# howardlau1999/pytorch-ddp-template

Hardware: NVIDIA H100
Metric: samples/sec (whole box, device-timed, max over ranks) for ResNet-50 DDP at 1/2/4/8 H100 (higher is better)
Workload: dtype bf16; 1 GPU; model=resnet50, global_batch=32, per_gpu_batch=32, image_size=224, parallelism=dp1, loss=mse(dense one-hot target), optimizer=sgd lr1e-3 + clip_grad_norm 1000 + linear warmup/decay, transport=single, cuda_graph=True

## Files before the change

b200ddp/csrc/conv_wgmma.cu:

```cuda
#include "conv.h"

#include <cuda.h>
#include <mutex>
#include <unordered_map>
#include <vector>

#include "drv.h"
#include "tc_primitives.cuh"

namespace b200 {
namespace {
using namespace tc;

constexpr int BLOCK_K = 64;
constexpr int UMMA_K = 16;
constexpr int kThreads = 256;
constexpr int kMmaWarps = 4;
constexpr int kMaxRing = 12;
constexpr int kSlabBytes = 128 * 128;
constexpr int kStagingBytes = 2 * kSlabBytes;
constexpr int kBarrierBytes = 1024;
constexpr int kTrStride = 36;
constexpr int kStatsScratchBytes = 4 * 32 * kTrStride * 4;
__host__ __device__ constexpr int acc_stride(int block_n) { return block_n + 8; }
__host__ __device__ constexpr int acc_bytes(int block_n) { return 128 * acc_stride(block_n) * 4; }

struct TapGemmParams {
  int M_total, Kc, Nc;
  int R, S, pad;
  int mirror;
  int mode;
  int H, W;
  int BH, BI, tiles_h, Wp;
  int num_m_tiles, num_n_tiles;
  int dense_rows;
  int a_chunk_bytes;
  int KC, TB;
  int s_stage_bytes, s_stages, b_slot_bytes, b_stages;
  uint32_t a_tx_bytes;
  int set_base_offset;
  int b_tap_stride;
  int row_mul;
  int b_resident;
  int chunk_stride;
  float* col_stats;
  const __nv_bfloat16* addend;
  const __nv_bfloat16* bn_x;
  const uint8_t* bn_mask;
  const float* bn_mean;
  const float* bn_rstd;
  long long* dbg;
};

__device__ __forceinline__ void tma_load_4d(const CUtensorMap* map, uint64_t* bar, void* smem, int c0, int c1, int c2, int c3) {
  asm volatile(
      "cp.async.bulk.tensor.4d.shared::cluster.global.mbarrier::complete_tx::bytes [%0], [%1, {%3, %4, %5, %6}], [%2];"
      ::"r"(smem_u32(smem)), "l"(reinterpret_cast<uint64_t>(map)), "r"(smem_u32(bar)), "r"(c0), "r"(c1), "r"(c2), "r"(c3) : "memory");
}
__device__ __forceinline__ void bulk_wait_read_all() { asm volatile("cp.async.bulk.wait_group.read 0;" ::: "memory"); }
__device__ __forceinline__ void epi_bar_sync() { asm volatile("bar.sync 1, 128;" ::: "memory"); }

__device__ __forceinline__ uint64_t make_desc_rowoff(uint32_t addr, uint32_t lbo, uint32_t sbo, int set_base_offset) {
  uint64_t d = make_smem_desc(addr, lbo, sbo);
  if (set_base_offset) d |= (uint64_t)((addr >> 7) & 7u) << 49;
  return d;
}

__device__ __forceinline__ bool acc_row_to_dense(const TapGemmParams& p, int i, int* dense) {
  if (p.mode == 2) {
    const int h = i / p.Wp, w = i - h * p.Wp;
    *dense = h * p.W + w;
    return h < p.BH && w < p.W;
  }
  *dense = i;
  return i < p.dense_rows;
}

__device__ __forceinline__ float warp_column_sum32(const float* v, float* tr, int lane) {
#pragma unroll
  for (int q = 0; q < 8; ++q)
    *reinterpret_cast<float4*>(tr + lane * kTrStride + 4 * q) = make_float4(v[4 * q], v[4 * q + 1], v[4 * q + 2], v[4 * q + 3]);
  __syncwarp();
  float s = 0.f;
#pragma unroll
  for (int r = 0; r < 32; ++r) s += tr[r * kTrStride + lane];
  __syncwarp();
  return s;
}

__device__ __forceinline__ bool elect_one() {
  uint32_t pred;
  asm volatile("{\n\t.reg .pred P;\n\telect.sync _|P, 0xFFFFFFFF;\n\tselp.u32 %0, 1, 0, P;\n\t}" : "=r"(pred));
  return pred != 0;
}

template <int BLOCK_N, bool B_MN, int EPI>
__global__ void __launch_bounds__(kThreads, 1)
conv_tap_gemm_kernel(const __grid_constant__ CUtensorMap map_a, const __grid_constant__ CUtensorMap map_b,
                     const __grid_constant__ CUtensorMap map_d, const TapGemmParams p) {
  constexpr int kBBytes = BLOCK_N * BLOCK_K * 2;
  constexpr int kAccStride = acc_stride(BLOCK_N);
  extern __shared__ uint8_t smem_raw[];
  uint8_t* smem = reinterpret_cast<uint8_t*>((reinterpret_cast<uintptr_t>(smem_raw) + 1023) & ~uintptr_t(1023));
  uint8_t* s_ring = smem;
  uint8_t* b_ring = s_ring + p.s_stages * p.s_stage_bytes;
  uint8_t* staging = b_ring + p.b_stages * p.b_slot_bytes;
  [[maybe_unused]] float* stats_scratch = reinterpret_cast<float*>(staging + kStagingBytes);
  float* acc_smem = reinterpret_cast<float*>(staging + kStagingBytes + (EPI != 0 ? kStatsScratchBytes : 0));
  uint64_t* s_full = reinterpret_cast<uint64_t*>(reinterpret_cast<uint8_t*>(acc_smem) + acc_bytes(BLOCK_N));
  uint64_t* s_empty = s_full + kMaxRing;
  uint64_t* b_full = s_empty + kMaxRing;
  uint64_t* b_empty = b_full + kMaxRing;

  const int warp = threadIdx.x >> 5, lane = threadIdx.x & 31;
  const long long t_begin = clock64();
  const int num_tiles = p.num_m_tiles * p.num_n_tiles;
  const int cblocks = p.Kc / BLOCK_K;
  const int taps = p.R * p.S;
  const int chunks_per_tile = cblocks * taps;

  if (warp == 0 && lane == 0) { tma_prefetch_desc(&map_a); tma_prefetch_desc(&map_b); tma_prefetch_desc(&map_d); }
  if (warp == 1) {
    if (lane < kMaxRing) {
      mbar_init(&s_full[lane], (p.mode == 2 || p.b_resident) ? 1 : 2); mbar_init(&s_empty[lane], kMmaWarps);
      mbar_init(&b_full[lane], 1); mbar_init(&b_empty[lane], kMmaWarps);
    }
    asm volatile("fence.mbarrier_init.release.cluster;" ::: "memory");
  }
  __syncthreads();
#define B200_T0 if (dbg) t = clock64();
#define B200_T1(acc) if (dbg) acc += clock64() - t;

  if (warp == 0 || warp == 3) {
    const bool is_a = (warp == 0);
    int ss = 0, bs = 0;
    uint32_t sph = 0, bph = 0;
    long long d_w = 0, d_i = 0, t = 0;
    const bool dbg = p.dbg != nullptr && blockIdx.x == 0;
    if constexpr (!B_MN) {
      if (!is_a && p.b_resident) {
        if (elect_one()) {
          mbar_expect_tx(&b_full[0], (uint32_t)chunks_per_tile * kBBytes);
          int cb_i = 0, r_i = 0, s_i = 0;
          for (int q = 0; q < chunks_per_tile; ++q) {
            tma_load_2d(&map_b, &b_full[0], b_ring + q * kBBytes, (r_i * p.S + s_i) * p.b_tap_stride + cb_i * BLOCK_K, 0);
            if (++s_i == p.S) { s_i = 0; if (++r_i == p.R) { r_i = 0; ++cb_i; } }
          }
        }
        __syncwarp();
      }
    }
    for (int tile = blockIdx.x; tile < num_tiles; tile += gridDim.x) {
      const int mt = tile / p.num_n_tiles, nt = tile - mt * p.num_n_tiles;
      const int n0 = nt * BLOCK_N;
      int img0 = 0, h0 = 0;
      if (p.mode != 0) { img0 = (mt / p.tiles_h) * p.BI; h0 = (mt % p.tiles_h) * p.BH; }
      if (p.mode != 2) {
        if (!is_a && p.b_resident) continue;
        int cb = 0, r = 0, sx = 0;
        for (int q0 = 0; q0 < chunks_per_tile; q0 += p.KC) {
          B200_T0 mbar_wait(&s_empty[ss], sph ^ 1); B200_T1(d_w)
          B200_T0
          if (elect_one()) {
            uint8_t* dst = s_ring + ss * p.s_stage_bytes;
            int cb_i = cb, r_i = r, s_i = sx;
            if (is_a) {
              mbar_expect_tx(&s_full[ss], (uint32_t)p.KC * p.a_tx_bytes);
              for (int j = 0; j < p.KC; ++j) {
                if (p.mode == 0) {
                  tma_load_4d(&map_a, &s_full[ss], dst, cb_i * BLOCK_K, mt * 128, 0, 0);
                } else {
                  const int dh = p.mirror ? p.pad - r_i : r_i - p.pad, dw = p.mirror ? p.pad - s_i : s_i - p.pad;
                  tma_load_4d(&map_a, &s_full[ss], dst, cb_i * BLOCK_K, dw, h0 * p.row_mul + dh, img0);
                }
                dst += p.chunk_stride;
                if (++s_i == p.S) { s_i = 0; if (++r_i == p.R) { r_i = 0; ++cb_i; } }
              }
            } else {
              mbar_expect_tx(&s_full[ss], (uint32_t)p.KC * kBBytes);
              for (int j = 0; j < p.KC; ++j) {
                uint8_t* sb = dst + p.a_chunk_bytes;
                const int bcol = (r_i * p.S + s_i) * p.b_tap_stride;
                if constexpr (!B_MN) {
                  tma_load_2d(&map_b, &s_full[ss], sb, bcol + cb_i * BLOCK_K, n0);
                } else {
#pragma unroll
                  for (int c = 0; c < BLOCK_N / 64; ++c)
                    tma_load_2d(&map_b, &s_full[ss], sb + c * (64 * BLOCK_K * 2), bcol + n0 + 64 * c, cb_i * BLOCK_K);
                }
                dst += p.chunk_stride;
                if (++s_i == p.S) { s_i = 0; if (++r_i == p.R) { r_i = 0; ++cb_i; } }
              }
            }
          }
          __syncwarp();
          for (int j = 0; j < p.KC; ++j) { if (++sx == p.S) { sx = 0; if (++r == p.R) { r = 0; ++cb; } } }
          if (++ss == p.s_stages) { ss = 0; sph ^= 1; }
          B200_T1(d_i)
        }
      } else if (is_a) {
        for (int cb = 0; cb < cblocks; ++cb) {
          B200_T0 mbar_wait(&s_empty[ss], sph ^ 1); B200_T1(d_w)
          B200_T0
          if (elect_one()) {
            mbar_expect_tx(&s_full[ss], p.a_tx_bytes);
            tma_load_4d(&map_a, &s_full[ss], s_ring + ss * p.s_stage_bytes, cb * BLOCK_K, -p.pad, h0 - p.pad, img0);
          }
          __syncwarp();
          if (++ss == p.s_stages) { ss = 0; sph ^= 1; }
          B200_T1(d_i)
        }
      } else {
        for (int cb = 0; cb < cblocks; ++cb) {
          for (int tap0 = 0; tap0 < taps; tap0 += p.TB) {
            B200_T0 mbar_wait(&b_empty[bs], bph ^ 1); B200_T1(d_w)
            B200_T0
            if (elect_one()) {
              mbar_expect_tx(&b_full[bs], (uint32_t)p.TB * kBBytes);
              for (int j = 0; j < p.TB; ++j) {
                uint8_t* sb = b_ring + bs * p.b_slot_bytes + j * kBBytes;
                const int bcol = (tap0 + j) * p.b_tap_stride;
                if constexpr (!B_MN) {
                  tma_load_2d(&map_b, &b_full[bs], sb, bcol + cb * BLOCK_K, n0);
                } else {
#pragma unroll
                  for (int c = 0; c < BLOCK_N / 64; ++c)
                    tma_load_2d(&map_b, &b_full[bs], sb + c * (64 * BLOCK_K * 2), bcol + n0 + 64 * c, cb * BLOCK_K);
                }
              }
            }
            __syncwarp();
            if (++bs == p.b_stages) { bs = 0; bph ^= 1; }
            B200_T1(d_i)
          }
        }
      }
    }
    if (dbg && lane == 0) { p.dbg[is_a ? 0 : 2] = d_w; p.dbg[is_a ? 1 : 3] = d_i; }
  } else if (warp >= 4) {
    constexpr int kTB = B_MN ? 1 : 0;
    constexpr uint32_t kLboB = B_MN ? BLOCK_K * 128 : 16;
    constexpr uint32_t kStepB = B_MN ? UMMA_K * 128 : UMMA_K * 2;
    constexpr uint64_t kHalfA = (64 * 128) >> 4;
    const uint64_t a_desc0 = make_smem_desc(smem_u32(s_ring), 16, 1024);
    const uint64_t b_desc_s0 = make_smem_desc(smem_u32(s_ring), kLboB, 1024);
    const uint64_t b_desc_b0 = make_smem_desc(smem_u32(b_ring), kLboB, 1024);
    const int ew = warp - 4;
    const bool t0 = (ew == 0 && lane == 0);
    int ss = 0, bs = 0;
    uint32_t sph = 0, bph = 0, slab = 0;
    long long d_wf = 0, d_mma = 0, d_ep = 0, t = 0;
    const bool dbg = p.dbg != nullptr && blockIdx.x == 0 && t0;
    [[maybe_unused]] float st_s[BLOCK_N / 32], st_q[BLOCK_N / 32];
    constexpr bool STATS = (EPI != 0);
    [[maybe_unused]] float* tr = stats_scratch + ew * (32 * kTrStride);
    if constexpr (STATS) {
#pragma unroll
      for (int i = 0; i < BLOCK_N / 32; ++i) { st_s[i] = 0.f; st_q[i] = 0.f; }
    }
    if (p.b_resident) mbar_wait(&b_full[0], 0);
    for (int tile = blockIdx.x; tile < num_tiles; tile += gridDim.x) {
      WgAcc<BLOCK_N> acc;
      uint32_t acc_on = 0;
      if (p.mode != 2) {
        for (int q0 = 0; q0 < chunks_per_tile; q0 += p.KC) {
          B200_T0 mbar_wait(&s_full[ss], sph); B200_T1(d_wf)
          B200_T0
          wgmma_fence();
          uint32_t off = (uint32_t)(ss * p.s_stage_bytes);
          for (int j = 0; j < p.KC; ++j) {
            const uint64_t da = a_desc0 + (uint64_t)(off >> 4);
            const uint64_t db = p.b_resident ? b_desc_b0 + (uint64_t)(((uint32_t)(q0 + j) * (uint32_t)kBBytes) >> 4)
                                             : b_desc_s0 + (uint64_t)((off + p.a_chunk_bytes) >> 4);
#pragma unroll
            for (int k = 0; k < BLOCK_K / UMMA_K; ++k) {
              const uint64_t dak = da + (uint64_t)(k * ((UMMA_K * 2) >> 4));
              wgmma_tile<BLOCK_N, 0, kTB>(acc, dak, dak + kHalfA, db + (uint64_t)(k * (kStepB >> 4)), acc_on);
              acc_on = 1;
            }
            off += (uint32_t)p.chunk_stride;
          }
          wgmma_commit();
          wgmma_wait<0>();
          __syncwarp();
          if (lane == 0) mbar_arrive(&s_empty[ss]);
          if (++ss == p.s_stages) { ss = 0; sph ^= 1; }
          B200_T1(d_mma)
        }
      } else {
        for (int cb = 0; cb < cblocks; ++cb) {
          B200_T0 mbar_wait(&s_full[ss], sph); B200_T1(d_wf)
          const uint32_t a_off = (uint32_t)(ss * p.s_stage_bytes);
          for (int tap0 = 0; tap0 < taps; tap0 += p.TB) {
            B200_T0 mbar_wait(&b_full[bs], bph); B200_T1(d_wf)
            B200_T0
            wgmma_fence();
            int r = tap0 / p.S, sx = tap0 - r * p.S;
            for (int j = 0; j < p.TB; ++j) {
              const int rr = p.mirror ? (p.R - 1 - r) : r, sc = p.mirror ? (p.S - 1 - sx) : sx;
              const uint64_t da = make_desc_rowoff(smem_u32(s_ring) + a_off + (uint32_t)(rr * p.Wp + sc) * 128u, 16, 1024, p.set_base_offset);
              const uint64_t db = b_desc_b0 + (uint64_t)((uint32_t)(bs * p.b_slot_bytes + j * kBBytes) >> 4);
#pragma unroll
              for (int k = 0; k < BLOCK_K / UMMA_K; ++k) {
                const uint64_t dak = da + (uint64_t)(k * ((UMMA_K * 2) >> 4));
                wgmma_tile<BLOCK_N, 0, kTB>(acc, dak, dak + kHalfA, db + (uint64_t)(k * (kStepB >> 4)), acc_on);
                acc_on = 1;
              }
              if (++sx == p.S) { sx = 0; ++r; }
            }
            wgmma_commit();
            wgmma_wait<0>();
            __syncwarp();
            if (lane == 0) {
              mbar_arrive(&b_empty[bs]);
              if (tap0 + p.TB >= taps) mbar_arrive(&s_empty[ss]);
            }
            if (++bs == p.b_stages) { bs = 0; bph ^= 1; }
            B200_T1(d_mma)
          }
          if (++ss == p.s_stages) { ss = 0; sph ^= 1; }
        }
      }
      B200_T0
      const int mt = tile / p.num_n_tiles, nt = tile - mt * p.num_n_tiles;
      const int n0 = nt * BLOCK_N;
      int row0;
      if (p.mode == 0) row0 = mt * 128;
      else row0 = (((mt / p.tiles_h) * p.BI) * p.H + (mt % p.tiles_h) * p.BH) * p.W;
      int dense;
      bool valid = acc_row_to_dense(p, ew * 32 + lane, &dense);
      valid = valid && (row0 + dense < p.M_total);
      wg_bar_sync();
      acc_to_smem<BLOCK_N>(acc, acc_smem, kAccStride, threadIdx.x - 128);
      wg_bar_sync();
#pragma unroll
      for (int c = 0; c < BLOCK_N; c += 64) {
        if (n0 + c >= p.Nc) break;
        uint8_t* buf = staging + (slab & 1u) * kSlabBytes;
        const uint32_t buf_s = smem_u32(buf);
#pragma unroll
        for (int half = 0; half < 2; ++half) {
          uint32_t rr[32];
          acc_row_ld32(acc_smem, kAccStride, ew * 32 + lane, c + 32 * half, rr);
          if constexpr (EPI == 1) {
            float sv[32], qv[32];
#pragma unroll
            for (int i = 0; i < 32; ++i) {
              const float v = __bfloat162float(__float2bfloat16_rn(__uint_as_float(rr[i])));
              sv[i] = valid ? v : 0.f;
              qv[i] = sv[i] * sv[i];
            }
            const float cs = warp_column_sum32(sv, tr, lane);
            const float cq = warp_column_sum32(qv, tr, lane);
            const int ci = (c >> 5) + half;
#pragma unroll
            for (int i = 0; i < BLOCK_N / 32; ++i)
              if (i == ci) { st_s[i] += cs; st_q[i] += cq; }
          }
          if constexpr (EPI == 2) {
            const int col0 = n0 + c + 32 * half;
            const size_t grow = (size_t)(row0 + dense);
            float v[32];
#pragma unroll
            for (int i = 0; i < 32; ++i) v[i] = __uint_as_float(rr[i]);
            if (p.addend != nullptr && valid) {
              const uint4* ap = reinterpret_cast<const uint4*>(p.addend + grow * p.Nc + col0);
#pragma unroll
              for (int q = 0; q < 4; ++q) {
                const uint4 raw = __ldg(ap + q);
                const __nv_bfloat162* h = reinterpret_cast<const __nv_bfloat162*>(&raw);
#pragma unroll
                for (int j = 0; j < 4; ++j) { const float2 f = __bfloat1622float2(h[j]); v[8 * q + 2 * j] += f.x; v[8 * q + 2 * j + 1] += f.y; }
              }
            }
#pragma unroll
            for (int i = 0; i < 32; ++i) { v[i] = __bfloat162float(__float2bfloat16_rn(v[i])); rr[i] = __float_as_uint(v[i]); }
            if (p.bn_x != nullptr) {
              float sv[32], qv[32];
              uint32_t mk = 0xffffffffu;
              float xv[32];
              if (valid) {
                const uint4* xp = reinterpret_cast<const uint4*>(p.bn_x + grow * p.Nc + col0);
#pragma unroll
                for (int q = 0; q < 4; ++q) {
                  const uint4 raw = __ldg(xp + q);
                  const __nv_bfloat162* h = reinterpret_cast<const __nv_bfloat162*>(&raw);
#pragma unroll
                  for (int j = 0; j < 4; ++j) { const float2 f = __bfloat1622float2(h[j]); xv[8 * q + 2 * j] = f.x; xv[8 * q + 2 * j + 1] = f.y; }
                }
                if (p.bn_mask != nullptr) mk = __ldg(reinterpret_cast<const uint32_t*>(p.bn_mask + grow * (size_t)(p.Nc >> 3) + (col0 >> 3)));
              } else {
                mk = 0u;
#pragma unroll
                for (int i = 0; i < 32; ++i) xv[i] = 0.f;
              }
              const float my_mean = (col0 + lane < p.Nc) ? __ldg(p.bn_mean + col0 + lane) : 0.f;
              const float my_rstd = (col0 + lane < p.Nc) ? __ldg(p.bn_rstd + col0 + lane) : 0.f;
#pragma unroll
              for (int i = 0; i < 32; ++i) {
                const float mean_i = __shfl_sync(0xffffffffu, my_mean, i), rstd_i = __shfl_sync(0xffffffffu, my_rstd, i);
                const float dyp = ((mk >> i) & 1u) ? v[i] : 0.f;
                sv[i] = dyp;
                qv[i] = dyp * (xv[i] - mean_i) * rstd_i;
              }
              const float cs = warp_column_sum32(sv, tr, lane);
              const float cq = warp_column_sum32(qv, tr, lane);
              const int ci = (c >> 5) + half;
#pragma unroll
              for (int i = 0; i < BLOCK_N / 32; ++i)
                if (i == ci) { st_s[i] += cs; st_q[i] += cq; }
            }
          }
          if (valid) {
#pragma unroll
            for (int q = 0; q < 4; ++q) {
              __nv_bfloat162 h[4];
#pragma unroll
              for (int j = 0; j < 4; ++j) h[j] = __floats2bfloat162_rn(__uint_as_float(rr[8 * q + 2 * j]), __uint_as_float(rr[8 * q + 2 * j + 1]));
              const int chunk = half * 4 + q;
              const uint32_t* w = reinterpret_cast<const uint32_t*>(h);
              asm volatile("st.shared.v4.b32 [%0], {%1, %2, %3, %4};"
                           ::"r"(buf_s + (uint32_t)(dense * 128 + ((chunk ^ (dense & 7)) << 4))), "r"(w[0]), "r"(w[1]), "r"(w[2]), "r"(w[3]) : "memory");
            }
          }
        }
        fence_async_smem();
        if (t0) bulk_wait_read_all();
        epi_bar_sync();
        if (t0) { tma_store_2d(&map_d, buf, n0 + c, row0); bulk_commit(); }
        ++slab;
      }
      B200_T1(d_ep)
    }
    if (dbg) { p.dbg[5] = d_wf; p.dbg[6] = d_mma; p.dbg[9] = d_ep; }
    if (STATS && p.col_stats != nullptr) {
      float* comb = stats_scratch;
      epi_bar_sync();
#pragma unroll
      for (int i = 0; i < BLOCK_N / 32; ++i) {
        comb[(ew * 2 + 0) * BLOCK_N + 32 * i + lane] = st_s[i];
        comb[(ew * 2 + 1) * BLOCK_N + 32 * i + lane] = st_q[i];
      }
      epi_bar_sync();
      const int nt = blockIdx.x % p.num_n_tiles;
      const size_t g = (size_t)(blockIdx.x / p.num_n_tiles), G = (size_t)(gridDim.x / p.num_n_tiles);
      for (int j = ew * 32 + lane; j < 2 * BLOCK_N; j += 128) {
        const int which = j / BLOCK_N, cc = j - which * BLOCK_N;
        const int col = nt * BLOCK_N + cc;
        if (col < p.Nc) {
          const float v = ((comb[(0 * 2 + which) * BLOCK_N + cc] + comb[(1 * 2 + which) * BLOCK_N + cc]) + comb[(2 * 2 + which) * BLOCK_N + cc]) +
                          comb[(3 * 2 + which) * BLOCK_N + cc];
          p.col_stats[((size_t)which * G + g) * p.Nc + col] = v;
        }
      }
    }
    if (t0) bulk_wait_all();
  }

  __syncthreads();
  if (p.dbg != nullptr && blockIdx.x == 0 && threadIdx.x == 0) p.dbg[10] = clock64() - t_begin;
}
#undef B200_T0
#undef B200_T1

struct MapKey {
  const void* ptr; uint64_t d[4]; uint64_t s[3]; uint32_t b[4]; int rank;
  bool operator==(const MapKey& o) const {
    if (ptr != o.ptr || rank != o.rank) return false;
    for (int i = 0; i < 4; ++i) if (d[i] != o.d[i] || b[i] != o.b[i]) return false;
    for (int i = 0; i < 3; ++i) if (s[i] != o.s[i]) return false;
    return true;
  }
};
struct MapKeyHash {
  size_t operator()(const MapKey& k) const {
    size_t h = std::hash<const void*>()(k.ptr) ^ (size_t)k.rank;
    for (int i = 0; i < 4; ++i) h = (h * 1000003u) ^ (size_t)k.d[i] ^ ((size_t)k.b[i] << 20);
    for (int i = 0; i < 3; ++i) h = (h * 1000003u) ^ (size_t)k.s[i];
    return h;
  }
};

}

CUtensorMap conv_encode_map(const void* ptr, int rank, const uint64_t* dims, const uint64_t* strides, const uint32_t* box) {
  static std::mutex mu;
  static std::unordered_map<MapKey, CUtensorMap, MapKeyHash> cache;
  MapKey key{};
  key.ptr = ptr; key.rank = rank;
  for (int i = 0; i < rank; ++i) { key.d[i] = dims[i]; key.b[i] = box[i]; }
  for (int i = 0; i + 1 < rank; ++i) key.s[i] = strides[i];
  {
    std::lock_guard<std::mutex> g(mu);
    auto it = cache.find(key);
    if (it != cache.end()) return it->second;
  }
  auto& drv = Driver::get();
  if (!drv.TensorMapEncodeTiled) throw std::runtime_error("conv: cuTensorMapEncodeTiled unavailable");
  static thread_local bool ctx_bound = false;
  if (!ctx_bound) { B200_CUDA_CHECK(cudaFree(nullptr)); ctx_bound = true; }
  CUtensorMap map;
  cuuint64_t d[4], s[3];
  cuuint32_t b[4], es[4] = {1, 1, 1, 1};
  for (int i = 0; i < rank; ++i) { d[i] = dims[i]; b[i] = box[i]; }
  for (int i = 0; i + 1 < rank; ++i) s[i] = strides[i];
  B200_DRV_CHECK(drv.TensorMapEncodeTiled(&map, CU_TENSOR_MAP_DATA_TYPE_BFLOAT16, rank, const_cast<void*>(ptr), d, s, b, es,
                                          CU_TENSOR_MAP_INTERLEAVE_NONE, CU_TENSOR_MAP_SWIZZLE_128B, CU_TENSOR_MAP_L2_PROMOTION_L2_256B,
                                          CU_TENSOR_MAP_FLOAT_OOB_FILL_NONE));
  std::lock_guard<std::mutex> g(mu);
  if (cache.size() > 8192) cache.clear();
  cache.emplace(key, map);
  return map;
}

bool conv_tile_plan(int N, int H, int W, int R, int S, int want_mode, ConvTilePlan* plan) {
  ConvTilePlan pl;
  const int taps = R * S;
  if (taps == 1) {
    if (want_mode > 0) return false;
    pl.mode = 0;
    pl.num_m_tiles = ceil_div((long long)N * H * W, 128);
    pl.dense_rows = 128; pl.acc_rows = 128; pl.a_rows = 128;
    *plan = pl;
    return true;
  }
  if (R != 3 || S != 3) return false;
  auto halo = [&]() {
    const int Wp = W + 2;
    int bh = 0;
    for (int d = 1; d <= H; ++d)
      if (H % d == 0 && d * Wp <= 128 && (d + 2) * Wp <= 256 * 1) bh = d;
    if (bh == 0 || Wp > 256 || bh + 2 > 256) return false;
    pl.mode = 2; pl.BH = bh; pl.BI = 1; pl.tiles_h = H / bh; pl.Wp = Wp;
    pl.num_m_tiles = N * pl.tiles_h;
    pl.dense_rows = bh * W; pl.acc_rows = bh * Wp; pl.a_rows = (bh + 2) * Wp;
    return true;
  };
  auto patch = [&]() {
    if (W > 128) return false;
    int bh = 0;
    for (int d = 1; d <= H; ++d)
      if (H % d == 0 && W * d <= 128) bh = d;
    if (bh == 0) return false;
    int bi = 1;
    if (bh == H)
      for (int d = 1; d <= N; ++d)
        if (N % d == 0 && W * H * d <= 128) bi = d;
    pl.mode = 1; pl.BH = bh; pl.BI = bi; pl.tiles_h = H / bh; pl.Wp = W;
    pl.num_m_tiles = (N / bi) * pl.tiles_h;
    pl.dense_rows = W * bh * bi; pl.acc_rows = pl.dense_rows; pl.a_rows = pl.dense_rows;
    return true;
  };
  bool ok;
  if (want_mode == 1) ok = patch();
  else if (want_mode == 2) ok = halo();
  else ok = halo() || patch();
  if (!ok) return false;
  *plan = pl;
  return true;
}

int conv_grid_size(int num_m_tiles, int num_n_tiles, bool stats) {
  const long long tiles = (long long)num_m_tiles * num_n_tiles;
  int grid = tiles < kNumSMs ? (int)tiles : kNumSMs;
  if (stats && num_n_tiles > 1) {
    grid = (grid / num_n_tiles) * num_n_tiles;
    if (grid < num_n_tiles) grid = num_n_tiles;
  }
  return grid;
}

int conv_pick_block_n(int Nc, int num_m_tiles, int want) {
  (void)num_m_tiles;
  if (want == 256) return 128;
  if (want != 0) return want;
  return Nc % 128 != 0 ? 64 : 128;
}

int conv_stat_groups(int N, int H, int W, int Cin, int Cout, int R, int S, const ConvLaunchCfg& cfg) {
  ConvTilePlan pl;
  int mode = cfg.mode;
  if (mode < 0 && R == 3) mode = (Cin == 64) ? 2 : 1;
  if (!conv_tile_plan(N, H, W, R, S, mode, &pl)) return 0;
  const int bn = conv_pick_block_n(Cout, pl.num_m_tiles, cfg.block_n);
  const int nn = ceil_div(Cout, bn);
  return conv_grid_size(pl.num_m_tiles, nn, true) / nn;
}

namespace {

template <int BLOCK_N, bool B_MN, int EPI>
void launch_variant(const CUtensorMap& ma, const CUtensorMap& mb, const CUtensorMap& md, TapGemmParams p, int want_kc, cudaStream_t stream) {
  constexpr int kBBytes = BLOCK_N * BLOCK_K * 2;
  const int budget = 227 * 1024 - kStagingBytes - kBarrierBytes - 1024 - (EPI != 0 ? kStatsScratchBytes : 0) - acc_bytes(BLOCK_N);
  const int taps = p.R * p.S;
  if (p.mode != 2) {
    const int chunks_per_tile = (p.Kc / BLOCK_K) * taps;
    if (p.b_resident && (B_MN || p.num_n_tiles != 1)) throw std::runtime_error("conv: a resident filter needs a K-major filter and one n-tile");
    p.chunk_stride = p.a_chunk_bytes + (p.b_resident ? 0 : kBBytes);
    p.b_slot_bytes = p.b_resident ? chunks_per_tile * kBBytes : 0;
    p.b_stages = p.b_resident ? 1 : 0;
    const int chunk = p.chunk_stride;
    const int ring_budget = budget - p.b_stages * p.b_slot_bytes;
    int kc = want_kc > 0 ? want_kc : 2;
    while (kc > 1 && (chunks_per_tile % kc != 0 || ring_budget / (kc * chunk) < 3)) --kc;
    p.KC = kc; p.TB = 1;
    p.s_stage_bytes = kc * chunk;
    p.s_stages = ring_budget / p.s_stage_bytes;
    if (p.s_stages > kMaxRing) p.s_stages = kMaxRing;
    if (p.s_stages < 2) throw std::runtime_error("conv: shared memory budget exceeded");
  } else {
    p.KC = 1; p.chunk_stride = 0; p.b_resident = 0;
    p.s_stage_bytes = p.a_chunk_bytes;
    int s_st = 0, b_st = 0;
    for (int tb = 3; tb >= 1; tb -= 2) {
      if (tb == 3 && (3 * kBBytes > 48 * 1024 || taps % 3 != 0)) continue;
      p.TB = tb;
      p.b_slot_bytes = p.TB * kBBytes;
      const int groups = taps / p.TB;
      s_st = budget / (p.s_stage_bytes + groups * p.b_slot_bytes);
      if (s_st < 2) s_st = 2;
      if (s_st > kMaxRing) s_st = kMaxRing;
      b_st = (budget - s_st * p.s_stage_bytes) / p.b_slot_bytes;
      if (b_st > kMaxRing) b_st = kMaxRing;
      if (b_st >= 2) break;
    }
    if (b_st < 2) throw std::runtime_error("conv: shared memory budget exceeded");
    p.s_stages = s_st; p.b_stages = b_st;
  }
  const int smem = p.s_stages * p.s_stage_bytes + p.b_stages * p.b_slot_bytes + kStagingBytes + kBarrierBytes + 1024 + (EPI != 0 ? kStatsScratchBytes : 0) +
                   acc_bytes(BLOCK_N);
  auto kernel = conv_tap_gemm_kernel<BLOCK_N, B_MN, EPI>;
  static std::atomic<unsigned long long> configured{0};
  ensure_max_dynamic_smem(kernel, 227 * 1024, configured);
  const int grid = conv_grid_size(p.num_m_tiles, p.num_n_tiles, EPI != 0);
  kernel<<<grid, kThreads, smem, stream>>>(ma, mb, md, p);
  B200_CUDA_CHECK(cudaGetLastError()); B200_COUNT_LAUNCH(1);
}

}

void launch_conv_tap_gemm(const void* a, const void* w, void* d, int N, int H, int W, int Cin, int Cout, int R, int S, bool dgrad,
                          const ConvLaunchCfg& cfg, float* col_stats, cudaStream_t stream, const ConvBwdFusion* fuse) {
  const int Kc = dgrad ? Cout : Cin, Nc = dgrad ? Cin : Cout;
  if (Kc % BLOCK_K != 0 || Nc % 64 != 0) throw std::runtime_error("conv: channel counts must be multiples of 64");
  if (R != S || (R != 1 && R != 3)) throw std::runtime_error("conv: 1x1 or 3x3 filters");
  if (dgrad && fuse == nullptr && col_stats != nullptr) throw std::runtime_error("conv: column statistics ride on the forward pass only");
  if (fuse != nullptr && !dgrad) throw std::runtime_error("conv: the BatchNorm-backward fusion rides on the data gradient");
  if (fuse != nullptr && fuse->bn_x != nullptr && col_stats == nullptr) throw std::runtime_error("conv: fused BatchNorm backward needs the partial-sum workspace");
  ConvTilePlan pl;
  int mode = cfg.mode;
  if (mode < 0 && R == 3) mode = (Kc == 64) ? 2 : 1;
  if (!conv_tile_plan(N, H, W, R, S, mode, &pl)) throw std::runtime_error("conv: no tile plan for this geometry");
  const long long M_total = (long long)N * H * W;
  TapGemmParams p{};
  p.M_total = (int)M_total; p.Kc = Kc; p.Nc = Nc;
  p.R = R; p.S = S; p.pad = (R - 1) / 2;
  p.mirror = dgrad ? 1 : 0;
  p.mode = pl.mode;
  p.H = H; p.W = W; p.BH = pl.BH; p.BI = pl.BI; p.tiles_h = pl.tiles_h; p.Wp = pl.Wp;
  p.num_m_tiles = pl.num_m_tiles;
  p.dense_rows = pl.dense_rows;
  p.a_tx_bytes = (uint32_t)(pl.a_rows * 128);
  p.a_chunk_bytes = ((pl.a_rows * 128 + 1023) / 1024) * 1024;
  if (p.a_chunk_bytes < 128 * 128) p.a_chunk_bytes = 128 * 128;
  p.set_base_offset = cfg.set_base_offset;
  p.b_tap_stride = Cin;
  p.row_mul = 1;
  p.b_resident = 0;
  p.col_stats = col_stats;
  p.addend = fuse ? reinterpret_cast<const __nv_bfloat16*>(fuse->addend) : nullptr;
  p.bn_x = fuse ? reinterpret_cast<const __nv_bfloat16*>(fuse->bn_x) : nullptr;
  p.bn_mask = fuse ? reinterpret_cast<const uint8_t*>(fuse->bn_mask) : nullptr;
  p.bn_mean = fuse ? fuse->bn_mean : nullptr;
  p.bn_rstd = fuse ? fuse->bn_rstd : nullptr;
  p.dbg = reinterpret_cast<long long*>(cfg.debug_counters);
  const int block_n = conv_pick_block_n(Nc, pl.num_m_tiles, cfg.block_n);
  if (block_n != 64 && block_n != 128) throw std::runtime_error("conv: block_n must be 0 (auto), 64, 128 or 256 (runs as two 128-wide n-tiles)");
  p.num_n_tiles = ceil_div(Nc, block_n);

  CUtensorMap ma;
  if (pl.mode == 0) {
    uint64_t dm[4] = {(uint64_t)Kc, (uint64_t)M_total, 1, 1};
    uint64_t st[3] = {(uint64_t)Kc * 2, (uint64_t)Kc * 2 * (uint64_t)M_total, (uint64_t)Kc * 2 * (uint64_t)M_total};
    uint32_t bx[4] = {64, 128, 1, 1};
    ma = conv_encode_map(a, 4, dm, st, bx);
  } else {
    uint64_t dm[4] = {(uint64_t)Kc, (uint64_t)W, (uint64_t)H, (uint64_t)N};
    uint64_t st[3] = {(uint64_t)Kc * 2, (uint64_t)W * Kc * 2, (uint64_t)H * W * Kc * 2};
    uint32_t bx[4] = {64, (uint32_t)(pl.mode == 2 ? pl.Wp : W), (uint32_t)(pl.mode == 2 ? pl.BH + 2 : pl.BH), (uint32_t)pl.BI};
    ma = conv_encode_map(a, 4, dm, st, bx);
  }
  CUtensorMap mb;
  {
    uint64_t dm[2] = {(uint64_t)R * S * Cin, (uint64_t)Cout};
    uint64_t st[1] = {(uint64_t)R * S * Cin * 2};
    uint32_t bx[2] = {64, (uint32_t)(dgrad ? 64 : block_n)};
    mb = conv_encode_map(w, 2, dm, st, bx);
  }
  CUtensorMap md;
  {
    uint64_t dm[2] = {(uint64_t)Nc, (uint64_t)M_total};
    uint64_t st[1] = {(uint64_t)Nc * 2};
    uint32_t bx[2] = {64, (uint32_t)pl.dense_rows};
    md = conv_encode_map(d, 2, dm, st, bx);
  }
#define B200_CONV_DISPATCH(BN)                                                                         \
  if (block_n == BN) {                                                                                 \
    if (dgrad && fuse != nullptr) launch_variant<BN, true, 2>(ma, mb, md, p, cfg.kc, stream);          \
    else if (dgrad) launch_variant<BN, true, 0>(ma, mb, md, p, cfg.kc, stream);                        \
    else if (col_stats != nullptr) launch_variant<BN, false, 1>(ma, mb, md, p, cfg.kc, stream);        \
    else launch_variant<BN, false, 0>(ma, mb, md, p, cfg.kc, stream);                                  \
    return;                                                                                            \
  }
  B200_CONV_DISPATCH(64)
  B200_CONV_DISPATCH(128)
#undef B200_CONV_DISPATCH
}

int stem_stat_groups(int N, int H, int W) {
  StemGeom g;
  if (!stem_geom(H, W, &g)) return 0;
  return conv_grid_size(N * g.Ho, 1, true);
}

void launch_stem_conv_fprop(const void* xp, const void* w2, void* y, int N, int H, int W, int Cout, float* col_stats, bool resident_filter,
                            void* debug_counters, cudaStream_t stream) {
  StemGeom g;
  if (!stem_geom(H, W, &g)) throw std::runtime_error("stem conv: unsupported image size");
  if (Cout != 64) throw std::runtime_error("stem conv: 64 output channels");
  const long long M_total = (long long)N * g.Ho * g.Wo;
  TapGemmParams p{};
  p.M_total = (int)M_total; p.Kc = 64; p.Nc = Cout;
  p.R = kStemTaps; p.S = 1; p.pad = 0; p.mirror = 0;
  p.mode = 1;
  p.H = g.Ho; p.W = g.Wo; p.BH = 1; p.BI = 1; p.tiles_h = g.Ho; p.Wp = g.Wo;
  p.num_m_tiles = N * g.Ho;
  p.num_n_tiles = 1;
  p.dense_rows = g.Wo;
  p.a_tx_bytes = (uint32_t)(g.Wo * 128);
  p.a_chunk_bytes = 128 * 128;
  p.b_tap_stride = 64;
  p.row_mul = 1;
  p.b_resident = resident_filter ? 1 : 0;
  p.col_stats = col_stats;
  p.dbg = reinterpret_cast<long long*>(debug_counters);
  const uint64_t row_pitch = (uint64_t)g.Wp * 16;
  CUtensorMap ma, mb, md;
  {
    uint64_t dm[4] = {64, (uint64_t)g.Wo, (uint64_t)g.Hp2, (uint64_t)N};
    uint64_t st[3] = {32, row_pitch, row_pitch * (uint64_t)g.Hp2};
    uint32_t bx[4] = {64, (uint32_t)g.Wo, 1, 1};
    ma = conv_encode_map(xp, 4, dm, st, bx);
  }
  {
    uint64_t dm[2] = {(uint64_t)kStemK, (uint64_t)Cout};
    uint64_t st[1] = {(uint64_t)kStemK * 2};
    uint32_t bx[2] = {64, 64};
    mb = conv_encode_map(w2, 2, dm, st, bx);
  }
  {
    uint64_t dm[2] = {(uint64_t)Cout, (uint64_t)M_total};
    uint64_t st[1] = {(uint64_t)Cout * 2};
    uint32_t bx[2] = {64, (uint32_t)g.Wo};
    md = conv_encode_map(y, 2, dm, st, bx);
  }
  if (col_stats != nullptr) launch_variant<64, false, 1>(ma, mb, md, p, 0, stream);
  else launch_variant<64, false, 0>(ma, mb, md, p, 0, stream);
}

}
```

b200ddp/models/resnet.py:

```python
from __future__ import annotations

import os
from typing import List

import torch
import torch.nn as nn

from ..ops import Conv3x3, FusedBatchNormAct2d, Linear, MaxPool3x3s2, PointwiseConv2d, StemConv7x7
from ..ops.bottleneck import bottleneck_forward, bottleneck_native_ok


class Bottleneck(nn.Module):
    expansion = 4

    def __init__(self, inplanes: int, planes: int, stride: int = 1, downsample: nn.Module | None = None):
        super().__init__()
        self.conv1 = PointwiseConv2d(inplanes, planes)
        self.bn1 = FusedBatchNormAct2d(planes, relu=True)
        self.conv2 = Conv3x3(planes, planes, stride=stride)
        self.bn2 = FusedBatchNormAct2d(planes, relu=True)
        self.conv3 = PointwiseConv2d(planes, planes * self.expansion)
        self.bn3 = FusedBatchNormAct2d(planes * self.expansion, relu=True)
        self.downsample = downsample

    def forward(self, x):
        if os.environ.get("B200DDP_BLOCK_FUSE", "0") == "1" and bottleneck_native_ok(self, x):
            return bottleneck_forward(self, x)
        if self.downsample is None:
            identity = x
        else:
            y, part = self.downsample[0].forward_with_stats(x)
            identity = self.downsample[1](y, partials=part)
        y, part = self.conv1.forward_with_stats(x)
        out = self.bn1(y, partials=part)
        y, part = self.conv2.forward_with_stats(out)
        out = self.bn2(y, partials=part)
        y, part = self.conv3.forward_with_stats(out)
        return self.bn3(y, residual=identity, partials=part)


class ResNet(nn.Module):
    def __init__(self, layers: List[int], num_classes: int = 1000, zero_init_residual: bool = False):
        super().__init__()
        self.inplanes = 64
        self.conv1 = StemConv7x7(3, 64)
        self.bn1 = FusedBatchNormAct2d(64, relu=True)
        self.maxpool = MaxPool3x3s2()
        self.layer1 = self._make_layer(64, layers[0], 1)
        self.layer2 = self._make_layer(128, layers[1], 2)
        self.layer3 = self._make_layer(256, layers[2], 2)
        self.layer4 = self._make_layer(512, layers[3], 2)
        self.avgpool = nn.AdaptiveAvgPool2d((1, 1))
        self.fc = Linear(512 * Bottleneck.expansion, num_classes)
        for m in self.modules():
            if isinstance(m, nn.Conv2d):
                nn.init.kaiming_normal_(m.weight, mode="fan_out", nonlinearity="relu")
            elif isinstance(m, nn.BatchNorm2d):
                nn.init.ones_(m.weight)
                nn.init.zeros_(m.bias)
        if zero_init_residual:
            for m in self.modules():
                if isinstance(m, Bottleneck):
                    nn.init.zeros_(m.bn3.weight)

    def _make_layer(self, planes: int, blocks: int, stride: int) -> nn.Sequential:
        downsample = None
        if stride != 1 or self.inplanes != planes * Bottleneck.expansion:
            downsample = nn.Sequential(PointwiseConv2d(self.inplanes, planes * Bottleneck.expansion, stride=stride),
                                       FusedBatchNormAct2d(planes * Bottleneck.expansion))
        mods = [Bottleneck(self.inplanes, planes, stride, downsample)]
        self.inplanes = planes * Bottleneck.expansion
        mods += [Bottleneck(self.inplanes, planes) for _ in range(1, blocks)]
        return nn.Sequential(*mods)

    def forward(self, x):
        if self.training:
            y, part = self.conv1.forward_with_stats(x)
        else:
            y, part = self.conv1(x), None
        x = self.maxpool(self.bn1(y, partials=part))
        x = self.layer4(self.layer3(self.layer2(self.layer1(x))))
        x = torch.flatten(self.avgpool(x), 1)
        return self.fc(x)


def resnet50(num_classes: int = 1000, **kw) -> ResNet:
    return ResNet([3, 4, 6, 3], num_classes, **kw)


def resnet152(num_classes: int = 1000, **kw) -> ResNet:
    return ResNet([3, 8, 36, 3], num_classes, **kw)
```

b200ddp/ops/bottleneck.py:

```python
from __future__ import annotations

import torch

from .. import _ext
from . import functional as Fn


def _bn_args(bn):
    momentum = bn.momentum if bn.momentum is not None else 0.1
    return bn.running_mean, bn.running_var, bn.num_batches_tracked, bn.eps, momentum


class _BottleneckFn(torch.autograd.Function):
    @staticmethod
    def forward(ctx, x, w1, g1, b1, w2, g2, b2, w3, g3, b3, wd, gd, bd, block):
        C = _ext.get()
        cl = Fn._cl
        x = cl(x)
        w1c, w2c, w3c = cl(w1), cl(w2), cl(w3)
        y1, p1 = C.conv_fprop(x, w1c, 1, 0, -1, 0, 0, True)
        a1, s1, m1 = C.bn_forward_partials(y1, None, g1, b1, *_bn_args(block.bn1), True, p1)
        y2, p2 = C.conv_fprop(a1, w2c, 1, 1, -1, 0, 0, True)
        a2, s2, m2 = C.bn_forward_partials(y2, None, g2, b2, *_bn_args(block.bn2), True, p2)
        y3, p3 = C.conv_fprop(a2, w3c, 1, 0, -1, 0, 0, True)
        has_ds = wd is not None
        if has_ds:
            wdc = cl(wd)
            yd, pd = C.conv_fprop(x, wdc, 1, 0, -1, 0, 0, True)
            idn, sd, _ = C.bn_forward_partials(yd, None, gd, bd, *_bn_args(block.downsample[1]), False, pd)
        else:
            wdc = yd = sd = None
            idn = x
        out, s3, m3 = C.bn_forward_partials(y3, idn, g3, b3, *_bn_args(block.bn3), True, p3)
        ctx.save_for_backward(x, w1c, w2c, w3c, wdc, y1, a1, y2, a2, y3, yd, s1, s2, s3, sd, m1, m2, m3, g1, g2, g3, gd)
        ctx.block = block
        ctx.has_ds = has_ds
        ctx.strides = (w1.stride(), w3.stride(), wd.stride() if has_ds else None)
        return out

    @staticmethod
    def backward(ctx, dout):
        C = _ext.get()
        (x, w1, w2, w3, wd, y1, a1, y2, a2, y3, yd, s1, s2, s3, sd, m1, m2, m3, g1, g2, g3, gd) = ctx.saved_tensors
        blk = ctx.block
        dout = Fn._cl(dout)

        def wgrad(dy, inp, w, k, strides=None):
            n, cin, h, wdt = inp.shape
            if Fn._wgrad_native(cin, w.shape[0], k, n * h * wdt):
                dw = C.conv_wgrad(dy, inp, k, 1, (k - 1) // 2, 0, 0, 0)
            else:
                pad = (k - 1) // 2
                dw = torch.ops.aten.convolution_backward(dy, inp, w, None, [1, 1], [pad, pad], [1, 1], False, [0, 0], 1, [False, True, False])[1]
            if strides is not None and tuple(dw.stride()) != tuple(strides):
                dw = dw.as_strided(dw.shape, strides)
            return dw

        ws = blk.bn3._workspace(y3)
        dy3, dres, dp3 = C.bn_backward(dout, y3, m3, g3, s3, True, True, ws[2], ws[3])
        dw3 = wgrad(dy3, a2, w3, 1, ctx.strides[1])
        da2, part2 = C.conv_dgrad(dy3, w3, 1, 0, -1, 0, 0, 0, None, y2, m2, s2)
        dy2, _, dp2 = C.bn_backward_partials(da2, y2, m2, g2, s2, True, False, part2)
        dw2 = wgrad(dy2, a1, w2, 3)
        da1, part1 = C.conv_dgrad(dy2, w2, 1, 1, -1, 0, 0, 0, None, y1, m1, s1)
        dy1, _, dp1 = C.bn_backward_partials(da1, y1, m1, g1, s1, True, False, part1)
        dw1 = wgrad(dy1, x, w1, 1, ctx.strides[0])
        dwd = dgd = dbd = None
        if ctx.has_ds:
            wsd = blk.downsample[1]._workspace(yd)
            dyd, _, dpd = C.bn_backward(dres, yd, None, gd, sd, False, False, wsd[2], wsd[3])
            dwd = wgrad(dyd, x, wd, 1, ctx.strides[2])
            shortcut = C.conv_dgrad(dyd, wd, 1, 0, -1, 0, 0, 0)[0]
            dgd, dbd = dpd[0], dpd[1]
        else:
            shortcut = dres
        dx = C.conv_dgrad(dy1, w1, 1, 0, -1, 0, 0, 0, shortcut)[0] if ctx.needs_input_grad[0] else None
        return (dx, dw1, dp1[0], dp1[1], dw2, dp2[0], dp2[1], dw3, dp3[0], dp3[1], dwd, dgd, dbd, None)


def bottleneck_native_ok(block, x: torch.Tensor) -> bool:
    if not (x.is_cuda and block.training and torch.is_grad_enabled() and x.dim() == 4 and x.dtype == torch.bfloat16):
        return False
    convs = [block.conv1, block.conv2, block.conv3] + ([block.downsample[0]] if block.downsample is not None else [])
    bns = [block.bn1, block.bn2, block.bn3] + ([block.downsample[1]] if block.downsample is not None else [])
    xin = x
    for conv in convs:
        if not (conv.stride[0] == 1 and conv.weight.dtype == torch.bfloat16 and conv.in_channels % 64 == 0 and conv.out_channels % 64 == 0):
            return False
    if not Fn.conv_tc_supported(xin, block.conv1.weight, 1, 0):
        return False
    for bn in bns:
        if not (bn.track_running_stats and bn.weight is not None and bn.weight.dtype == torch.float32):
            return False
    return True


def bottleneck_forward(block, x: torch.Tensor) -> torch.Tensor:
    ds = block.downsample
    return _BottleneckFn.apply(x, block.conv1.weight, block.bn1.weight, block.bn1.bias, block.conv2.weight, block.bn2.weight, block.bn2.bias,
                               block.conv3.weight, block.bn3.weight, block.bn3.bias,
                               ds[0].weight if ds is not None else None, ds[1].weight if ds is not None else None,
                               ds[1].bias if ds is not None else None, block)
```

Before: 4566 samples/s.

## Overlap wgmma groups, stage accumulator per 64-column slab, add per-shape block-fuse gating

```diff
diff --git a/b200ddp/csrc/conv_wgmma.cu b/b200ddp/csrc/conv_wgmma.cu
--- a/b200ddp/csrc/conv_wgmma.cu
+++ b/b200ddp/csrc/conv_wgmma.cu
@@ -22,8 +22,24 @@
 constexpr int kBarrierBytes = 1024;
 constexpr int kTrStride = 36;
 constexpr int kStatsScratchBytes = 4 * 32 * kTrStride * 4;
-__host__ __device__ constexpr int acc_stride(int block_n) { return block_n + 8; }
-__host__ __device__ constexpr int acc_bytes(int block_n) { return 128 * acc_stride(block_n) * 4; }
+constexpr int kAccStride = 64 + 8;
+constexpr int kAccBytes = 128 * kAccStride * 4;
+
+template <int SLAB, int BN>
+__device__ __forceinline__ void acc_slab_to_smem(const WgAcc<BN>& acc, float* dst, int wg_thread) {
+  const int warp = wg_thread >> 5, lane = wg_thread & 31;
+  const int r0 = warp * 16 + (lane >> 2), c0 = 2 * (lane & 3);
+#pragma unroll
+  for (int half = 0; half < 2; ++half) {
+#pragma unroll
+    for (int j = 0; j < 8; ++j) {
+      const int q = 4 * (8 * SLAB + j);
+      float* p = dst + (half * 64 + r0) * kAccStride + 8 * j + c0;
+      *reinterpret_cast<float2*>(p) = make_float2(acc.h[half][q], acc.h[half][q + 1]);
+      *reinterpret_cast<float2*>(p + 8 * kAccStride) = make_float2(acc.h[half][q + 2], acc.h[half][q + 3]);
+    }
+  }
+}
 
 struct TapGemmParams {
   int M_total, Kc, Nc;
@@ -99,7 +115,6 @@
 conv_tap_gemm_kernel(const __grid_constant__ CUtensorMap map_a, const __grid_constant__ CUtensorMap map_b,
                      const __grid_constant__ CUtensorMap map_d, const TapGemmParams p) {
   constexpr int kBBytes = BLOCK_N * BLOCK_K * 2;
-  constexpr int kAccStride = acc_stride(BLOCK_N);
   extern __shared__ uint8_t smem_raw[];
   uint8_t* smem = reinterpret_cast<uint8_t*>((reinterpret_cast<uintptr_t>(smem_raw) + 1023) & ~uintptr_t(1023));
   uint8_t* s_ring = smem;
@@ -107,7 +122,7 @@
   uint8_t* staging = b_ring + p.b_stages * p.b_slot_bytes;
   [[maybe_unused]] float* stats_scratch = reinterpret_cast<float*>(staging + kStagingBytes);
   float* acc_smem = reinterpret_cast<float*>(staging + kStagingBytes + (EPI != 0 ? kStatsScratchBytes : 0));
-  uint64_t* s_full = reinterpret_cast<uint64_t*>(reinterpret_cast<uint8_t*>(acc_smem) + acc_bytes(BLOCK_N));
+  uint64_t* s_full = reinterpret_cast<uint64_t*>(reinterpret_cast<uint8_t*>(acc_smem) + kAccBytes);
   uint64_t* s_empty = s_full + kMaxRing;
   uint64_t* b_full = s_empty + kMaxRing;
   uint64_t* b_empty = b_full + kMaxRing;
@@ -262,6 +277,7 @@
     for (int tile = blockIdx.x; tile < num_tiles; tile += gridDim.x) {
       WgAcc<BLOCK_N> acc;
       uint32_t acc_on = 0;
+      int held_s = -1, held_b = -1;
       if (p.mode != 2) {
         for (int q0 = 0; q0 < chunks_per_tile; q0 += p.KC) {
           B200_T0 mbar_wait(&s_full[ss], sph); B200_T1(d_wf)
@@ -281,9 +297,10 @@
             off += (uint32_t)p.chunk_stride;
           }
           wgmma_commit();
-          wgmma_wait<0>();
+          wgmma_wait<1>();
           __syncwarp();
-          if (lane == 0) mbar_arrive(&s_empty[ss]);
+          if (lane == 0 && held_s >= 0) mbar_arrive(&s_empty[held_s]);
+          held_s = ss;
           if (++ss == p.s_stages) { ss = 0; sph ^= 1; }
           B200_T1(d_mma)
         }
@@ -309,17 +326,25 @@
               if (++sx == p.S) { sx = 0; ++r; }
             }
             wgmma_commit();
-            wgmma_wait<0>();
+            wgmma_wait<1>();
             __syncwarp();
-            if (lane == 0) {
-              mbar_arrive(&b_empty[bs]);
-              if (tap0 + p.TB >= taps) mbar_arrive(&s_empty[ss]);
-            }
+            if (lane == 0 && held_b >= 0) {
+              mbar_arrive(&b_empty[held_b]);
+              if (held_s >= 0) mbar_arrive(&s_empty[held_s]);
+            }
+            held_b = bs;
+            held_s = (tap0 + p.TB >= taps) ? ss : -1;
             if (++bs == p.b_stages) { bs = 0; bph ^= 1; }
             B200_T1(d_mma)
           }
           if (++ss == p.s_stages) { ss = 0; sph ^= 1; }
         }
+      }
+      wgmma_wait<0>();
+      __syncwarp();
+      if (lane == 0) {
+        if (held_b >= 0) mbar_arrive(&b_empty[held_b]);
+        if (held_s >= 0) mbar_arrive(&s_empty[held_s]);
       }
       B200_T0
       const int mt = tile / p.num_n_tiles, nt = tile - mt * p.num_n_tiles;
@@ -330,18 +355,19 @@
       int dense;
       bool valid = acc_row_to_dense(p, ew * 32 + lane, &dense);
       valid = valid && (row0 + dense < p.M_total);
-      wg_bar_sync();
-      acc_to_smem<BLOCK_N>(acc, acc_smem, kAccStride, threadIdx.x - 128);
-      wg_bar_sync();
 #pragma unroll
       for (int c = 0; c < BLOCK_N; c += 64) {
         if (n0 + c >= p.Nc) break;
+        wg_bar_sync();
+        if (c == 0) acc_slab_to_smem<0>(acc, acc_smem, threadIdx.x - 128);
+        else acc_slab_to_smem<BLOCK_N / 64 - 1>(acc, acc_smem, threadIdx.x - 128);
+        wg_bar_sync();
         uint8_t* buf = staging + (slab & 1u) * kSlabBytes;
         const uint32_t buf_s = smem_u32(buf);
 #pragma unroll
         for (int half = 0; half < 2; ++half) {
           uint32_t rr[32];
-          acc_row_ld32(acc_smem, kAccStride, ew * 32 + lane, c + 32 * half, rr);
+          acc_row_ld32(acc_smem, kAccStride, ew * 32 + lane, 32 * half, rr);
           if constexpr (EPI == 1) {
             float sv[32], qv[32];
 #pragma unroll
@@ -592,7 +618,7 @@
 template <int BLOCK_N, bool B_MN, int EPI>
 void launch_variant(const CUtensorMap& ma, const CUtensorMap& mb, const CUtensorMap& md, TapGemmParams p, int want_kc, cudaStream_t stream) {
   constexpr int kBBytes = BLOCK_N * BLOCK_K * 2;
-  const int budget = 227 * 1024 - kStagingBytes - kBarrierBytes - 1024 - (EPI != 0 ? kStatsScratchBytes : 0) - acc_bytes(BLOCK_N);
+  const int budget = 227 * 1024 - kStagingBytes - kBarrierBytes - 1024 - (EPI != 0 ? kStatsScratchBytes : 0) - kAccBytes;
   const int taps = p.R * p.S;
   if (p.mode != 2) {
     const int chunks_per_tile = (p.Kc / BLOCK_K) * taps;
@@ -629,7 +655,7 @@
     p.s_stages = s_st; p.b_stages = b_st;
   }
   const int smem = p.s_stages * p.s_stage_bytes + p.b_stages * p.b_slot_bytes + kStagingBytes + kBarrierBytes + 1024 + (EPI != 0 ? kStatsScratchBytes : 0) +
-                   acc_bytes(BLOCK_N);
+                   kAccBytes;
   auto kernel = conv_tap_gemm_kernel<BLOCK_N, B_MN, EPI>;
   static std::atomic<unsigned long long> configured{0};
   ensure_max_dynamic_smem(kernel, 227 * 1024, configured);
diff --git a/b200ddp/models/resnet.py b/b200ddp/models/resnet.py
--- a/b200ddp/models/resnet.py
+++ b/b200ddp/models/resnet.py
@@ -1,13 +1,12 @@
 from __future__ import annotations
 
-import os
 from typing import List
 
 import torch
 import torch.nn as nn
 
 from ..ops import Conv3x3, FusedBatchNormAct2d, Linear, MaxPool3x3s2, PointwiseConv2d, StemConv7x7
-from ..ops.bottleneck import bottleneck_forward, bottleneck_native_ok
+from ..ops.bottleneck import bottleneck_forward, bottleneck_native_ok, fuse_selected
 
 
 class Bottleneck(nn.Module):
@@ -24,7 +23,8 @@
         self.downsample = downsample
 
     def forward(self, x):
-        if os.environ.get("B200DDP_BLOCK_FUSE", "0") == "1" and bottleneck_native_ok(self, x):
+        if x.dim() == 4 and fuse_selected(x.shape[1], self.conv1.out_channels, x.shape[2], x.shape[3], x.shape[0]) \
+                and bottleneck_native_ok(self, x):
             return bottleneck_forward(self, x)
         if self.downsample is None:
             identity = x
diff --git a/b200ddp/ops/bottleneck.py b/b200ddp/ops/bottleneck.py
--- a/b200ddp/ops/bottleneck.py
+++ b/b200ddp/ops/bottleneck.py
@@ -1,9 +1,13 @@
 from __future__ import annotations
+
+import os
 
 import torch
 
 from .. import _ext
 from . import functional as Fn
+
+FUSED_BLOCKS: frozenset = frozenset()
 
 
 def _bn_args(bn):
@@ -78,6 +82,13 @@
         return (dx, dw1, dp1[0], dp1[1], dw2, dp2[0], dp2[1], dw3, dp3[0], dp3[1], dwd, dgd, dbd, None)
 
 
+def fuse_selected(cin: int, planes: int, h: int, w: int, n: int) -> bool:
+    mode = os.environ.get("B200DDP_BLOCK_FUSE", "auto")
+    if mode in ("0", "1"):
+        return mode == "1"
+    return (cin, planes, h, w, n) in FUSED_BLOCKS
+
+
 def bottleneck_native_ok(block, x: torch.Tensor) -> bool:
     if not (x.is_cuda and block.training and torch.is_grad_enabled() and x.dim() == 4 and x.dtype == torch.bfloat16):
         return False
```

Result: no change. 4556 samples/s, median of 6 (-0.2%).
